# Kelvin-ywc/LPI

Hardware: AMD Instinct MI355X
Metric: image-text pairs/sec fwd+bwd (ViT-B/16, bs256/GPU) (higher is better)
Workload: dtype bf16; 1 GPU; BASELINE.json configs[2]: ViT-B/16 dual encoder bs=256/GPU prompt_depth=3 r=4 P=16, fwd+bwd incl. DecomposedPrompt grads + SGD step; global_batch=256, image=224x224, towers=lock step, GEMMs of one layer op grouped in one launch, parallelism=dp1, weights=synthetic (numpy Philox, CLIP-init scales), frozen

## Files before the change

### lpi_amd/csrc/gemm256p.hip

```cpp
#include "gemm256x128_tile.h"

extern int g_lpi_tuning[16];

namespace {

constexpr int T256 = 256;
constexpr int ROWB = 128;
constexpr int HALF_BYTES = 128 * ROWB;
constexpr int BUF_BYTES = 4 * HALF_BYTES;
constexpr int NTHR = 512;
constexpr int OFF_A0 = 0, OFF_A1 = HALF_BYTES, OFF_B0 = 2 * HALF_BYTES, OFF_B1 = 3 * HALF_BYTES;
constexpr int STG = BUF_BYTES;
constexpr int LDS_P = 2 * BUF_BYTES;
constexpr int EPI_PLAIN16 = 100;
template <int EPI, bool SAVE_U> constexpr bool slices_ok() { return !(EPI == LPI_EPI_QUICKGELU && SAVE_U); }

struct PProb {
    const void* A; const void* B; void* C; const float* bias; const void* residual; void* aux;
    int N, K, lda, ldb, ldc, ldr, ldaux, tiles_m, tiles_n;
    int vb0;
    int bias_off;
    int group_m;
};
struct PGroup {
    PProb p[2];
    int nprob;
    int n_full;
    int tail_blocks;
    int reserved;
    float alpha;
};

#ifdef LPI_GEMM_STAMPS
__device__ unsigned long long g_gemm_stamps[1024][8];
#define GS_NOW() __builtin_amdgcn_s_memtime()
#endif

template <typename T, typename TC, int EPI, bool RES, bool SAVE_U>
__global__ __launch_bounds__(NTHR, 2) void gemm256p_kernel(const PGroup grp)
{
    extern __shared__ __attribute__((aligned(16))) char smem[];
    constexpr int EPC = Elem<T>::EPC;
    constexpr int BK = ROWB / (int)sizeof(T);
    const int tid = threadIdx.x;
    const int lane = tid & 63;
    const int wave = __builtin_amdgcn_readfirstlane(tid >> 6);
    const int wm = wave >> 2, wn = wave & 3;
    const int G = gridDim.x;
    int group_m = 1;
    const float alpha = grp.alpha;
    typedef typename AuxT<T>::type TA;
    typedef float f32x8 __attribute__((ext_vector_type(8)));
    constexpr bool LNE = EPI == LPI_EPI_LN || EPI == LPI_EPI_LN_QUICKGELU;
    constexpr bool SLICES = slices_ok<EPI, SAVE_U>();
    constexpr bool P16 = EPI == EPI_PLAIN16;
    constexpr int EPIX = P16 ? LPI_EPI_NONE : EPI;
    const T* A = nullptr; const T* B = nullptr; TC* C = nullptr;
    const float* bias = nullptr; const float* residual = nullptr; TA* aux = nullptr;
    int K = 0, lda = 0, ldb = 0, ldc = 0, ldr = 0, ldaux = 0, tiles_m = 1, tiles_n = 1, nwg = 0, vb0 = 0, bias_off = 0;
    unsigned a_off = 0, b_off = 0;
    const int srow = tid >> 3;
    const int schunk = (tid & 7) ^ ((tid >> 4) & 7);
    auto bind = [&](int pi) {
        const PProb& P = grp.p[pi];
        A = (const T*)P.A; B = (const T*)P.B; C = (TC*)P.C; bias = P.bias; residual = (const float*)P.residual; aux = (TA*)P.aux;
        K = P.K; lda = P.lda; ldb = P.ldb; ldc = P.ldc; ldr = P.ldr; ldaux = P.ldaux; tiles_m = P.tiles_m; tiles_n = P.tiles_n;
        nwg = tiles_m * tiles_n; vb0 = P.vb0; bias_off = P.bias_off; group_m = P.group_m;
        a_off = (unsigned)(((size_t)srow * lda + schunk * EPC) * sizeof(T));
        b_off = (unsigned)(((size_t)srow * ldb + schunk * EPC) * sizeof(T));
    };

    auto coords = [&](int vb, int& m0, int& n0) {
        const int q = nwg >> 3, r = nwg & 7, xcd = vb & 7, idx = vb >> 3;
        const int t = (xcd < r ? xcd * (q + 1) : r * (q + 1) + (xcd - r) * q) + idx;
        const int gm = SLICES ? (group_m & 0xffff) : group_m;
        const int group = t / (gm * tiles_n);
        const int first_m = group * gm;
        const int gsz = min(tiles_m - first_m, gm);
        const int in_group = t - group * gm * tiles_n;
        m0 = (first_m + in_group % gsz) * T256;
        n0 = (in_group / gsz) * T256;
        if constexpr (SLICES) {
            const int wrap = (group_m >> 16) * T256;
            if (wrap) {
                if (m0 >= wrap) { m0 -= wrap; n0 += tiles_n * T256; }
                if (m0 >= wrap) { m0 -= wrap; n0 += tiles_n * T256; }
            }
        }
    };

    const unsigned lds_w = __builtin_amdgcn_readfirstlane((unsigned)(uintptr_t)(__attribute__((address_space(3))) char*)smem + wave * 1024);
    auto glds16 = [&](const T* sbase, unsigned voff, unsigned lds_addr) {
        unsigned keep;
        asm volatile("s_mov_b32 %0, m0\n\ts_mov_b32 m0, %3\n\ts_nop 0\n\tglobal_load_lds_dwordx4 %1, %2\n\ts_mov_b32 m0, %0"
                     : "=&s"(keep) : "v"(voff), "s"(sbase), "s"(lds_addr) : "memory");
    };
#ifndef LPI_A_POLICY
#define LPI_A_POLICY ""
#endif
    auto glds16a = [&](const T* sbase, unsigned voff, unsigned lds_addr) {
        unsigned keep;
        asm volatile("s_mov_b32 %0, m0\n\ts_mov_b32 m0, %3\n\ts_nop 0\n\tglobal_load_lds_dwordx4 %1, %2" LPI_A_POLICY "\n\ts_mov_b32 m0, %0"
                     : "=&s"(keep) : "v"(voff), "s"(sbase), "s"(lds_addr) : "memory");
    };
    auto stage_A = [&](int m0, int kt, int h, int buf) {
        const T* sb = A + (size_t)(m0 + h * 128) * lda + (size_t)kt * BK;
        const int lo = buf * BUF_BYTES + (h ? OFF_A1 : OFF_A0);
        glds16a(sb, a_off, lds_w + lo);
        glds16a(sb + (size_t)64 * lda, a_off, lds_w + lo + 8192);
    };
    auto stage_B = [&](int n0, int kt, int h, int buf) {
        const T* sb = B + (size_t)(n0 + h * 128) * ldb + (size_t)kt * BK;
        const int lo = buf * BUF_BYTES + (h ? OFF_B1 : OFF_B0);
        glds16(sb, b_off, lds_w + lo);
        glds16(sb + (size_t)64 * ldb, b_off, lds_w + lo + 8192);
    };

    const int frow = lane & 15, fg = lane >> 4, fsw = frow >> 1;
    int foff[2];
#pragma unroll
    for (int ks = 0; ks < 2; ++ks) foff[ks] = frow * ROWB + (((ks << 2) | fg) ^ fsw) * 16;
    const int a_base = (wm * 64) * ROWB;
    const int b_base = (wn * 32) * ROWB;

    Chunk fa[4][2], fb0[2][2], fb1[2][2];
    f32x4 acc[2][2][2][4];
    auto read_A = [&](const char* half) {
#pragma unroll
        for (int mi = 0; mi < 4; ++mi)
#pragma unroll
            for (int ks = 0; ks < 2; ++ks) fa[mi][ks].u = *reinterpret_cast<const uint4*>(half + a_base + mi * 16 * ROWB + foff[ks]);
    };
    auto read_B = [&](Chunk (&fb)[2][2], const char* half) {
#pragma unroll
        for (int ni = 0; ni < 2; ++ni)
#pragma unroll
            for (int ks = 0; ks < 2; ++ks) fb[ni][ks].u = *reinterpret_cast<const uint4*>(half + b_base + ni * 16 * ROWB + foff[ks]);
    };
    auto mma_quadrant = [&](f32x4 (&c)[2][2][2][4], int nh, int mh, const Chunk (&fb)[2][2]) {
        __builtin_amdgcn_s_setprio(1);
#pragma unroll
        for (int ks = 0; ks < 2; ++ks)
#pragma unroll
            for (int ni = 0; ni < 2; ++ni)
#pragma unroll
                for (int mi = 0; mi < 4; ++mi) mma_chunk<T>(c[nh][ni][mh][mi], fb[ni][ks], fa[mi][ks]);
        __builtin_amdgcn_s_setprio(0);
    };
#define PHASE_SYNC_IN()                                   \
    asm volatile("s_waitcnt lgkmcnt(0)" ::: "memory");    \
    __builtin_amdgcn_s_barrier();                         \
    __builtin_amdgcn_sched_barrier(0)
#define PHASE_SYNC_OUT()                                  \
    __builtin_amdgcn_sched_barrier(0);                    \
    __builtin_amdgcn_s_barrier();                         \
    asm volatile("" ::: "memory")

    int nk = 0;
    constexpr bool LATE = RES || EPI == LPI_EPI_DQUICKGELU;
    constexpr bool SIDE16 = (RES && sizeof(TC) == 2) || EPI == LPI_EPI_DQUICKGELU;
    constexpr bool STATS = EPI == LPI_EPI_NONE && RES && SAVE_U && __is_same(TC, f16_t);
    constexpr int NST = 8 + (STATS ? 2 : 0);
    const char* side_base = nullptr;
    int side_ld = 0;
    float* const bias_lds = reinterpret_cast<float*>(smem + LDS_P);
    if constexpr (SIDE16) {
        for (int pi = 0; pi < grp.nprob; ++pi) {
            const float* bp = grp.p[pi].bias;
            float* dst = bias_lds + grp.p[pi].bias_off;
            for (int i = tid * 4; i < grp.p[pi].N; i += NTHR * 4)
                *reinterpret_cast<f32x4*>(dst + i) = bp ? *reinterpret_cast<const f32x4*>(bp + i) : f32x4{0.f, 0.f, 0.f, 0.f};
        }
        __syncthreads();
    }
    auto stage_side = [&](int m0, int n0, int p) {
        const char* sb = side_base + ((size_t)m0 * side_ld + n0) * 2;
        int l2 = lane;
        asm volatile("" : "+v"(l2));
#pragma unroll
        for (int i = 0; i < 4; ++i) {
            const int sr = 2 * (4 * wave + i) + (l2 >> 5);
            const int trow = (p >> 1) * 128 + (sr >> 5) * 64 + ((p & 1) * 2 + ((sr >> 4) & 1)) * 16 + (sr & 15);
            const unsigned voff = (unsigned)trow * (unsigned)side_ld * 2u + (unsigned)(l2 & 31) * 16u;
            unsigned keep;
            asm volatile("s_mov_b32 %0, m0\n\ts_mov_b32 m0, %3\n\ts_nop 0\n\tglobal_load_lds_dwordx4 %1, %2 nt\n\ts_mov_b32 m0, %0"
                         : "=&s"(keep) : "v"(voff), "s"(sb), "s"(lds_w + (p & 1) * 32768 + i * 1024 + wave * 3072) : "memory");
        }
    };

#ifdef LPI_GEMM_STAMPS
    unsigned long long gs_main = 0, gs_epi = 0, gs_next = 0, gs_tiles = 0, gs_t0 = 0, gs_t1 = 0, gs_t2 = 0;
    unsigned long long gs_e[4] = {0, 0, 0, 0}, gs_a = 0, gs_b = 0;
#endif
    const int n_full = grp.n_full;
    int vbv = blockIdx.x;
    bool lds_used = false;
    for (int pi = 0; pi < grp.nprob; ++pi) {
        bind(pi);
        nk = K / BK;
        if constexpr (SIDE16) {
            side_base = RES ? reinterpret_cast<const char*>(residual) : reinterpret_cast<const char*>(aux);
            side_ld = RES ? ldr : ldaux;
        }
        const int vend = min(vb0 + nwg, n_full);
        if (vbv < vb0) vbv += (vb0 - vbv + G - 1) / G * G;
        if (vbv >= vend) continue;
        if (lds_used) {
            asm volatile("s_waitcnt lgkmcnt(0)" ::: "memory");
            __builtin_amdgcn_s_barrier();
            asm volatile("" ::: "memory");
        }
        lds_used = true;
        int vb = vbv - vb0;
        const int lend = vend - vb0;
        int m0, n0;
        coords(vb, m0, n0);
        m0 = __builtin_amdgcn_readfirstlane(m0);
        n0 = __builtin_amdgcn_readfirstlane(n0);
        stage_A(m0, 0, 0, 0); stage_B(n0, 0, 0, 0); stage_B(n0, 0, 1, 0); stage_A(m0, 0, 1, 0);
        stage_A(m0, 1, 0, 1); stage_B(n0, 1, 0, 1); stage_B(n0, 1, 1, 1);
        asm volatile("s_waitcnt vmcnt(8)" ::: "memory");
        __builtin_amdgcn_s_barrier();
        bool first = true;
        for (;;) {
            const int nvb = vb + G;
            const bool more_tiles = nvb < lend;
            const bool has_next = more_tiles && !LATE;
            int nm0 = 0, nn0 = 0;
            if (more_tiles) coords(nvb, nm0, nn0);
            nm0 = __builtin_amdgcn_readfirstlane(nm0);
            nn0 = __builtin_amdgcn_readfirstlane(nn0);
#pragma unroll
            for (int a = 0; a < 2; ++a)
#pragma unroll
                for (int b = 0; b < 2; ++b)
#pragma unroll
                    for (int c = 0; c < 2; ++c)
#pragma unroll
                        for (int d = 0; d < 4; ++d) acc[a][b][c][d] = f32x4{0.f, 0.f, 0.f, 0.f};
            if (wm == 1) __builtin_amdgcn_s_barrier();

            auto ktile = [&](int kt, const int BUF, bool skip_wait) {
                const char* buf = smem + BUF * BUF_BYTES;
                const bool more1 = kt + 1 < nk, more2 = kt + 2 < nk;
                read_B(fb0, buf + OFF_B0);
                read_B(fb1, buf + OFF_B1);
                __builtin_amdgcn_sched_barrier(0);
                read_A(buf + OFF_A0);
                if (more1) {
                    stage_A(m0, kt + 1, 1, BUF ^ 1);
                    if (!skip_wait) asm volatile("s_waitcnt vmcnt(8)" ::: "memory");
                } else if (has_next) {
                    stage_A(nm0, 0, 1, BUF ^ 1);
                    asm volatile("s_waitcnt vmcnt(8)" ::: "memory");
                } else {
                    asm volatile("s_waitcnt vmcnt(0)" ::: "memory");
                    if constexpr (SIDE16) {
                        stage_side(m0, n0, 0);
                        stage_side(m0, n0, 1);
                    }
                }
                PHASE_SYNC_IN();
                mma_quadrant(acc, 0, 0, fb0);
                mma_quadrant(acc, 1, 0, fb1);
                PHASE_SYNC_OUT();
                read_A(buf + OFF_A1);
                if (more2) {
                    stage_A(m0, kt + 2, 0, BUF); stage_B(n0, kt + 2, 0, BUF); stage_B(n0, kt + 2, 1, BUF);
                    asm volatile("s_waitcnt vmcnt(8)" ::: "memory");
                } else if (more1) {
                    if (has_next) {
                        stage_A(nm0, 0, 0, BUF); stage_B(nn0, 0, 0, BUF); stage_B(nn0, 0, 1, BUF);
                        asm volatile("s_waitcnt vmcnt(8)" ::: "memory");
                    } else {
                        asm volatile("s_waitcnt vmcnt(2)" ::: "memory");
                    }
                } else if (!has_next && !SIDE16) {
                    asm volatile("s_waitcnt vmcnt(0)" ::: "memory");
                }
                PHASE_SYNC_IN();
                mma_quadrant(acc, 1, 1, fb1);
                mma_quadrant(acc, 0, 1, fb0);
                PHASE_SYNC_OUT();
            };
#ifdef LPI_GEMM_STAMPS
            gs_t0 = GS_NOW();
            if (gs_tiles) gs_next += gs_t0 - gs_t2;
#endif
            ktile(0, 0, !first);
            ktile(1, 1, false);
            for (int kt = 2; kt < nk; kt += 2) {
                ktile(kt, 0, false);
                ktile(kt + 1, 1, false);
            }
            if (wm == 0) __builtin_amdgcn_s_barrier();
#ifdef LPI_GEMM_STAMPS
            gs_t1 = GS_NOW();
            gs_main += gs_t1 - gs_t0;
#endif

            int lane_e = lane, wave_e = wave;
            asm volatile("" : "+v"(lane_e));
            asm volatile("" : "+s"(wave_e));
            const int lrow = lane_e & 15, lslot = lane_e >> 4;
            const int wm_e = wave_e >> 2, wn_e = wave_e & 3;
            if constexpr (P16) {
                typedef __attribute__((ext_vector_type(4))) unsigned u32x4_;
                const int l5 = lane_e & 31, lh = lane_e >> 5;
                TC* const cbase = C + (size_t)m0 * ldc + n0 + l5 * 8;
#pragma unroll
                for (int p = 0; p < 4; ++p) {
                    const int mh = p >> 1;
                    char* const sb = smem + STG + (p & 1) * 32768;
#pragma unroll
                    for (int mi2 = 0; mi2 < 2; ++mi2) {
                        const int s_row = wm_e * 32 + mi2 * 16 + lrow;
#pragma unroll
                        for (int nh = 0; nh < 2; ++nh)
#pragma unroll
                            for (int ni = 0; ni < 2; ++ni) {
                                const int c8 = nh * 32 + wn_e * 8 + ni * 4 + lslot;
                                const f32x4 a = acc[nh][ni][mh][(p & 1) * 2 + mi2] + 0.0f;
                                *reinterpret_cast<uint2*>(sb + s_row * 512 + ((c8 ^ (2 * lrow)) << 3)) = uint2{pack2_t<TC>(a[0], a[1]), pack2_t<TC>(a[2], a[3])};
                            }
                    }
                    asm volatile("s_waitcnt lgkmcnt(0)" ::: "memory");
                    __builtin_amdgcn_s_barrier();
                    asm volatile("" ::: "memory");
#pragma unroll
                    for (int i = 0; i < 4; ++i) {
                        const int s_row = wave_e * 8 + 2 * i + lh;
                        const int trow = mh * 128 + (s_row >> 5) * 64 + ((p & 1) * 2 + ((s_row >> 4) & 1)) * 16 + (s_row & 15);
                        const u32x4_ v = *reinterpret_cast<const u32x4_*>(sb + s_row * 512 + (((2 * l5) ^ (2 * (s_row & 15))) << 3));
                        if constexpr (LPI_NTC_DEFAULT) __builtin_nontemporal_store(v, reinterpret_cast<u32x4_*>(cbase + (size_t)trow * ldc));
                        else *reinterpret_cast<u32x4_*>(cbase + (size_t)trow * ldc) = v;
                    }
                    if (p == 1 && has_next) asm volatile("s_waitcnt vmcnt(8)" ::: "memory");
                }
            } else {
            const int ecol = n0 + lane_e * 4;
            f32x4 bv = f32x4{0.f, 0.f, 0.f, 0.f};
            if constexpr (SIDE16) bv = *reinterpret_cast<const f32x4*>(bias_lds + bias_off + ecol);
            else if (bias) bv = *reinterpret_cast<const f32x4*>(bias + ecol);
            f32x4 c1v = f32x4{0.f, 0.f, 0.f, 0.f};
            if constexpr (EPI == LPI_EPI_LN || EPI == LPI_EPI_LN_QUICKGELU) c1v = *reinterpret_cast<const f32x4*>(residual + 2 * (size_t)ldr + ecol);
            char* const stg = smem + STG;
#pragma unroll
            for (int p = 0; p < 4; ++p) {
                const int mh = p >> 1;
#ifdef LPI_GEMM_STAMPS
                gs_a = GS_NOW();
#endif
                if (p) {
                    asm volatile("s_waitcnt lgkmcnt(0)" ::: "memory");
                    __builtin_amdgcn_s_barrier();
                }
#ifdef LPI_GEMM_STAMPS
                gs_b = GS_NOW(); gs_e[0] += gs_b - gs_a;
#endif
                if constexpr (SIDE16) {
                    if (p >= 1 && p <= 2) stage_side(m0, n0, p + 1);
                    if (p == 3 && more_tiles) { stage_A(nm0, 0, 0, 0); stage_A(nm0, 0, 1, 0); }
                }
                f32x8 mu8, rs8;
                if constexpr (LNE) {
                    const int sr0 = wave_e * 8;
                    const int trow0 = mh * 128 + (sr0 >> 5) * 64 + ((p & 1) * 2 + ((sr0 >> 4) & 1)) * 16 + (sr0 & 15);
                    const float* pm = residual + (m0 + trow0);
                    const float* pr = pm + ldr;
                    asm volatile("s_load_dwordx8 %0, %2, 0x0\n\ts_load_dwordx8 %1, %3, 0x0" : "=&s"(mu8), "=&s"(rs8) : "s"(pm), "s"(pr));
                }
#pragma unroll
                for (int mi2 = 0; mi2 < 2; ++mi2) {
                    const int s_row = wm_e * 32 + mi2 * 16 + lrow;
#pragma unroll
                    for (int nh = 0; nh < 2; ++nh)
#pragma unroll
                        for (int ni = 0; ni < 2; ++ni) {
                            const int chunk = nh * 32 + wn_e * 8 + ni * 4 + lslot;
                            *reinterpret_cast<f32x4*>(stg + s_row * 1024 + ((chunk ^ (s_row & 7)) << 4)) = acc[nh][ni][mh][(p & 1) * 2 + mi2];
                        }
                }
                if constexpr (SIDE16) {
                    if (p == 0) asm volatile("s_waitcnt vmcnt(4)" ::: "memory");
                    else if (p == 3 && !more_tiles) asm volatile("s_waitcnt vmcnt(%0)" :: "n"(NST) : "memory");
                    else asm volatile("s_waitcnt vmcnt(%0)" :: "n"(NST + 4) : "memory");
                }
                if constexpr (LNE) asm volatile("s_waitcnt lgkmcnt(0)" : "+s"(mu8), "+s"(rs8) : : "memory");
                else asm volatile("s_waitcnt lgkmcnt(0)" ::: "memory");
#ifdef LPI_GEMM_STAMPS
                gs_a = GS_NOW(); gs_e[1] += gs_a - gs_b;
#endif
                __builtin_amdgcn_s_barrier();
                asm volatile("" ::: "memory");
#ifdef LPI_GEMM_STAMPS
                gs_b = GS_NOW(); gs_e[2] += gs_b - gs_a;
#endif
                float st_s[8], st_q[8];
#pragma unroll
                for (int rr = 0; rr < 8; ++rr) {
                    const int s_row = wave_e * 8 + rr;
                    const int trow = mh * 128 + (s_row >> 5) * 64 + ((p & 1) * 2 + ((s_row >> 4) & 1)) * 16 + (s_row & 15);
                    const f32x4 v = *reinterpret_cast<const f32x4*>(stg + s_row * 1024 + ((lane_e ^ (s_row & 7)) << 4));
                    if constexpr (SIDE16) {
                        f32x4 o = v * alpha + bv;
                        const char* sp = smem + (p & 1) * 32768 + s_row * 512 + lane_e * 8;
                        if constexpr (EPI == LPI_EPI_DQUICKGELU) {
                            const f32x4 u = Elem<TA>::ld4(reinterpret_cast<const TA*>(sp));
                            o *= u;
                        } else {
                            o += Elem<TC>::ld4(reinterpret_cast<const TC*>(sp));
                        }
                        if constexpr (STATS) {
                            const uint32_t w0 = pack2_t<f16_t>(o[0], o[1]), w1 = pack2_t<f16_t>(o[2], o[3]);
                            *reinterpret_cast<uint2*>(C + (size_t)(m0 + trow) * ldc + ecol) = uint2{w0, w1};
                            f16x4_sum_sumsq(w0, w1, st_s[rr], st_q[rr]);
                        } else {
                            if constexpr (LPI_NTC_DEFAULT && EPI == LPI_EPI_DQUICKGELU) st4_nt<TC>(C + (size_t)(m0 + trow) * ldc + ecol, o);
                            else Elem<TC>::st4(C + (size_t)(m0 + trow) * ldc + ecol, o);
                        }
                    } else {
                        gemm_epilogue_store<T, TC, EPI, RES, SAVE_U>(v, m0 + trow, ecol, C, ldc, bv, alpha, residual, ldr, aux, ldaux, c1v, LNE ? mu8[rr] : 0.f,
                                                                     LNE ? rs8[rr] : 1.f);
                    }
                }
                if constexpr (STATS) {
                    float so, qo;
                    rowstats8_half_reduce(st_s, st_q, lane_e, so, qo);
                    const int s_row = wave_e * 8 + ((lane_e >> 2) & 7);
                    const int trow = mh * 128 + (s_row >> 5) * 64 + ((p & 1) * 2 + ((s_row >> 4) & 1)) * 16 + (s_row & 15);
                    float* sp = reinterpret_cast<float*>(aux) + (size_t)(2 * ((n0 >> 7) + (lane_e >> 5))) * ldaux + (m0 + trow);
                    if ((lane_e & 3) == 0) { sp[0] = so; sp[ldaux] = qo; }
                }
#ifdef LPI_GEMM_STAMPS
                gs_a = GS_NOW(); gs_e[3] += gs_a - gs_b;
#endif
                if (p == 1 && has_next) asm volatile("s_waitcnt vmcnt(16)" ::: "memory");
                if constexpr (LATE && !SIDE16) {
                    if (p == 1 && more_tiles) {
                        stage_A(nm0, 0, 0, 0); stage_B(nn0, 0, 0, 0); stage_B(nn0, 0, 1, 0); stage_A(nm0, 0, 1, 0);
                    }
                    if (p == 3 && more_tiles) asm volatile("s_waitcnt vmcnt(16)" ::: "memory");
                }
            }
            }
#ifdef LPI_GEMM_STAMPS
            gs_t2 = GS_NOW();
            gs_epi += gs_t2 - gs_t1;
            ++gs_tiles;
#endif
            if (!more_tiles) { vbv = nvb + vb0; break; }
            asm volatile("s_waitcnt lgkmcnt(0)" ::: "memory");
            __builtin_amdgcn_s_barrier();
            asm volatile("" ::: "memory");
            vb = nvb; m0 = nm0; n0 = nn0;
            if constexpr (SIDE16) {
                stage_B(n0, 0, 0, 0); stage_B(n0, 0, 1, 0);
                stage_A(m0, 1, 0, 1); stage_B(n0, 1, 0, 1); stage_B(n0, 1, 1, 1);
                asm volatile("s_waitcnt vmcnt(6)" ::: "memory");
                __builtin_amdgcn_s_barrier();
            } else {
                stage_A(m0, 1, 0, 1); stage_B(n0, 1, 0, 1); stage_B(n0, 1, 1, 1);
                first = false;
            }
        }
    }
#undef PHASE_SYNC_IN
#undef PHASE_SYNC_OUT

#ifdef LPI_GEMM_STAMPS
    if (tid == 0 && blockIdx.x < 1024) {
        g_gemm_stamps[blockIdx.x][0] = gs_main; g_gemm_stamps[blockIdx.x][1] = gs_epi; g_gemm_stamps[blockIdx.x][2] = gs_next; g_gemm_stamps[blockIdx.x][3] = gs_tiles;
        for (int i = 0; i < 4; ++i) g_gemm_stamps[blockIdx.x][4 + i] = gs_e[i];
    }
#endif
    if (grp.tail_blocks > 0) {
        for (int j = blockIdx.x; j < grp.tail_blocks; j += G) {
            const int k = (j >> 4) * 8 + (j & 7), half = (j >> 3) & 1;
            const int v = n_full + k;
            const int pi = (grp.nprob > 1 && v >= grp.p[1].vb0) ? 1 : 0;
            bind(pi);
            const int lv = v - vb0;
            if (lv < 0 || lv >= nwg) continue;
            __syncthreads();
            int m0, n0;
            coords(lv, m0, n0);
            t128::tile<T, TC, EPIX, RES, SAVE_U>(m0, n0 + half * 128, K, A, lda, B, ldb, C, ldc, bias, residual, ldr, aux, ldaux, alpha, smem);
        }
    }
}

int cu_count_p() { return lpi_cu_count(); }

struct HostProb {
    int M, N, K;
    const void* A; int lda; const void* B; int ldb; void* C; int ldc; const float* bias; const float* residual; int ldr; void* aux; int ldaux;
};

template <typename T, typename TC, int EPI, bool RES, bool SAVE_U>
int launchp_impl(const HostProb* hp, int np, float alpha, hipStream_t s)
{
    constexpr bool SIDE16 = (RES && sizeof(TC) == 2) || EPI == LPI_EPI_DQUICKGELU;
    static_assert(EPI != EPI_PLAIN16 || (!RES && !SAVE_U && sizeof(TC) == 2), "EPI_PLAIN16: store-only, 2-byte output");
    const int ncu = cu_count_p();
    PGroup g = {};
    g.nprob = np;
    g.alpha = alpha;
    int v = 0, nsum = 0;
    for (int i = 0; i < np; ++i) {
        PProb& P = g.p[i];
        const HostProb& h = hp[i];
        P.A = h.A; P.B = h.B; P.C = h.C; P.bias = h.bias; P.residual = h.residual; P.aux = h.aux;
        P.N = h.N; P.K = h.K; P.lda = h.lda; P.ldb = h.ldb; P.ldc = h.ldc; P.ldr = h.ldr; P.ldaux = h.ldaux;
        P.tiles_m = h.M / T256; P.tiles_n = h.N / T256;
        P.vb0 = v;
        v += P.tiles_m * P.tiles_n;
        P.bias_off = nsum;
        P.group_m = g_lpi_tuning[4] > 0 ? g_lpi_tuning[4] : ((size_t)h.N * h.K * sizeof(T) <= ((size_t)5 << 20) ? 1 : 8);
        if (slices_ok<EPI, SAVE_U>() && P.group_m == 1 && g_lpi_tuning[15] >= 0 && P.tiles_m < 32768) {
            int S = 0;
            const size_t wbytes = (size_t)h.N * h.K * sizeof(T);
            if (g_lpi_tuning[15] > 0) S = g_lpi_tuning[15];
            else if (wbytes > ((size_t)3 << 20) && P.tiles_n % 2 == 0) S = 2;
            if ((S == 2 || S == 3) && P.tiles_n % S == 0 && P.tiles_n / S >= 2) {
                P.group_m |= P.tiles_m << 16;
                P.tiles_n /= S;
                P.tiles_m *= S;
            }
        }
        nsum += h.N;
    }
    if (SIDE16 && nsum > 8192) return LPI_ENOSYS;
    const int rem = v % ncu;
    g.n_full = v;
    if (g_lpi_tuning[6] != 0 && v - rem >= ncu && rem > 0 && rem <= ncu / 2 && (ncu % 8) == 0) {
        g.n_full = v - rem;
        g.tail_blocks = 16 * ((rem + 7) >> 3);
    }
    auto kern = gemm256p_kernel<T, TC, EPI, RES, SAVE_U>;
    const int LDS = std::max<int>(t128::LDS_BYTES, LDS_P + (SIDE16 ? nsum * 4 : 0));
    static LdsOnce once;
    if (int e = lpi_ensure_lds(once, (const void*)kern, 160 * 1024)) return e;
    lpi_note_gemm_kernel(g.tail_blocks ? LPI_GEMM_K_256_TAIL : LPI_GEMM_K_256);
    const int grid = std::min(ncu, std::max(g.n_full, g.tail_blocks));
    LPI_LAUNCH(kern, dim3(grid), dim3(NTHR), LDS, s, g);
    LPI_CHECK_LAST();
    return 0;
}

template <typename T, typename TC>
int dispatchp(int epi, const HostProb* hp, int np, float alpha, hipStream_t s)
{
    const bool res = hp[0].residual != nullptr, ax = hp[0].aux != nullptr;
    for (int i = 1; i < np; ++i)
        if ((hp[i].residual != nullptr) != res || (hp[i].aux != nullptr) != ax) return LPI_EINVAL;
    switch (epi) {
    case LPI_EPI_NONE:
        if (res) return launchp_impl<T, TC, LPI_EPI_NONE, true, false>(hp, np, alpha, s);
        if constexpr (sizeof(TC) == 2) {
            bool plain = alpha == 1.0f && !ax && g_lpi_tuning[14] != 1;
            for (int i = 0; i < np; ++i) plain = plain && hp[i].bias == nullptr;
            if (plain) return launchp_impl<T, TC, EPI_PLAIN16, false, false>(hp, np, alpha, s);
        }
        return launchp_impl<T, TC, LPI_EPI_NONE, false, false>(hp, np, alpha, s);
    case LPI_EPI_RES_ROWSTATS:
        if constexpr (sizeof(TC) == 2 && !__is_same(TC, bf16_t)) {
            if (!res || !ax) return LPI_EINVAL;
            return launchp_impl<T, TC, LPI_EPI_NONE, true, true>(hp, np, alpha, s);
        }
        return LPI_ENOSYS;
    case LPI_EPI_QUICKGELU:
        if (res) return LPI_ENOSYS;
        if (ax) return launchp_impl<T, TC, LPI_EPI_QUICKGELU, false, true>(hp, np, alpha, s);
        return launchp_impl<T, TC, LPI_EPI_QUICKGELU, false, false>(hp, np, alpha, s);
    case LPI_EPI_DQUICKGELU:
        if (res) return LPI_ENOSYS;
        if (!ax) return LPI_EINVAL;
        return launchp_impl<T, TC, LPI_EPI_DQUICKGELU, false, false>(hp, np, alpha, s);
    }
    return LPI_EINVAL;
}

template <typename T, typename TC>
int dispatchp_ln(int epi, const HostProb* hp, int np, float alpha, hipStream_t s)
{
    const bool ax = hp[0].aux != nullptr;
    for (int i = 0; i < np; ++i)
        if (!hp[i].residual || (hp[i].aux != nullptr) != ax) return LPI_EINVAL;
    if (epi == LPI_EPI_LN) {
        if (ax) return LPI_EINVAL;
        return launchp_impl<T, TC, LPI_EPI_LN, false, false>(hp, np, alpha, s);
    }
    if (ax) return launchp_impl<T, TC, LPI_EPI_LN_QUICKGELU, false, true>(hp, np, alpha, s);
    return launchp_impl<T, TC, LPI_EPI_LN_QUICKGELU, false, false>(hp, np, alpha, s);
}

int launch_group(int dtype, int c_dtype, int epilogue, const HostProb* hp, int np, float alpha, hipStream_t s)
{
    if (epilogue == LPI_EPI_LN || epilogue == LPI_EPI_LN_QUICKGELU) {
        if (dtype == LPI_F16 && c_dtype == LPI_BF16) return dispatchp_ln<f16_t, bf16_t>(epilogue, hp, np, alpha, s);
        if (dtype == LPI_F16 && c_dtype == LPI_F16) return dispatchp_ln<f16_t, f16_t>(epilogue, hp, np, alpha, s);
        if (dtype == LPI_BF16 && c_dtype == LPI_BF16) return dispatchp_ln<bf16_t, bf16_t>(epilogue, hp, np, alpha, s);
        return LPI_ENOSYS;
    }
    if (dtype == LPI_BF16 && c_dtype == LPI_BF16) return dispatchp<bf16_t, bf16_t>(epilogue, hp, np, alpha, s);
    if (dtype == LPI_BF16 && c_dtype == LPI_F32) return dispatchp<bf16_t, float>(epilogue, hp, np, alpha, s);
    if (dtype == LPI_BF16 && c_dtype == LPI_F16 && (epilogue == LPI_EPI_NONE || epilogue == LPI_EPI_RES_ROWSTATS) && hp[0].residual) {
        for (int i = 1; i < np; ++i) if (!hp[i].residual) return LPI_EINVAL;
        if (epilogue == LPI_EPI_RES_ROWSTATS) {
            for (int i = 0; i < np; ++i) if (!hp[i].aux) return LPI_EINVAL;
            return launchp_impl<bf16_t, f16_t, LPI_EPI_NONE, true, true>(hp, np, alpha, s);
        }
        return launchp_impl<bf16_t, f16_t, LPI_EPI_NONE, true, false>(hp, np, alpha, s);
    }
    if (dtype == LPI_F16 && c_dtype == LPI_F16) return dispatchp<f16_t, f16_t>(epilogue, hp, np, alpha, s);
    if (dtype == LPI_F16 && c_dtype == LPI_F32) return dispatchp<f16_t, float>(epilogue, hp, np, alpha, s);
    return LPI_ENOSYS;
}

}

#ifdef LPI_GEMM_STAMPS
extern "C" int lpi_gemm_stamps_read(unsigned long long* dst) {
    return (int)hipMemcpyFromSymbol(dst, HIP_SYMBOL(g_gemm_stamps), sizeof(unsigned long long) * 1024 * 8, 0, hipMemcpyDeviceToHost);
}
#endif

int lpi_gemm256p_launch(int dtype, int c_dtype, int M, int N, int K, const void* A, int lda, const void* B, int ldb, void* C, int ldc,
                        const float* bias, const float* residual, int ldr, int epilogue, void* aux, int ldaux, float alpha, hipStream_t s)
{
    const HostProb hp = {M, N, K, A, lda, B, ldb, C, ldc, bias, residual, ldr, aux, ldaux};
    return launch_group(dtype, c_dtype, epilogue, &hp, 1, alpha, s);
}

int lpi_gemm256p_launch2(int dtype, int c_dtype, int epilogue, float alpha, const lpi_gemm_desc* d, hipStream_t s)
{
    HostProb hp[2];
    for (int i = 0; i < 2; ++i)
        hp[i] = HostProb{d[i].M, d[i].N, d[i].K, d[i].A, d[i].lda, d[i].B, d[i].ldb, d[i].C, d[i].ldc, d[i].bias, (const float*)d[i].residual, d[i].ldr,
                         d[i].aux, d[i].ldaux};
    return launch_group(dtype, c_dtype, epilogue, hp, 2, alpha, s);
}
```

Before: 11410 pairs/s.

## Load residual/aux side tiles into registers and prefetch next tile during SIDE16 epilogue

Residual and dQuickGELU side inputs used to be staged through LDS with global_load_lds. They are now loaded straight into registers with nontemporal loads, spread across the last k-tile, the post-mainloop point and the epilogue rows. The SIDE16 path no longer uses the LATE schedule, so the next tile's A/B operands prefetch during the main loop as in the plain path, and the separate restage-and-barrier at tile change is dropped. The k-loop is restructured with explicit position tags, and bias loading into LDS is skipped when there is no bias. The changes aim to hide side-input latency and cut barriers and LDS traffic, at the cost of extra VGPRs (16 u32x2 per thread) and hand-tuned vmcnt counts that must exactly match the new load order.

```diff
diff --git a/lpi_amd/csrc/gemm256p.hip b/lpi_amd/csrc/gemm256p.hip
--- a/lpi_amd/csrc/gemm256p.hip
+++ b/lpi_amd/csrc/gemm256p.hip
@@ -157,35 +157,32 @@
     asm volatile("" ::: "memory")
 
     int nk = 0;
-    constexpr bool LATE = RES || EPI == LPI_EPI_DQUICKGELU;
+    constexpr bool LATE = RES && sizeof(TC) == 4;
     constexpr bool SIDE16 = (RES && sizeof(TC) == 2) || EPI == LPI_EPI_DQUICKGELU;
     constexpr bool STATS = EPI == LPI_EPI_NONE && RES && SAVE_U && __is_same(TC, f16_t);
     constexpr int NST = 8 + (STATS ? 2 : 0);
+    constexpr int NSL = SIDE16 ? 8 : 0;
     const char* side_base = nullptr;
     int side_ld = 0;
     float* const bias_lds = reinterpret_cast<float*>(smem + LDS_P);
     if constexpr (SIDE16) {
         for (int pi = 0; pi < grp.nprob; ++pi) {
             const float* bp = grp.p[pi].bias;
+            if (!bp) continue;
             float* dst = bias_lds + grp.p[pi].bias_off;
-            for (int i = tid * 4; i < grp.p[pi].N; i += NTHR * 4)
-                *reinterpret_cast<f32x4*>(dst + i) = bp ? *reinterpret_cast<const f32x4*>(bp + i) : f32x4{0.f, 0.f, 0.f, 0.f};
+            for (int i = tid * 4; i < grp.p[pi].N; i += NTHR * 4) *reinterpret_cast<f32x4*>(dst + i) = *reinterpret_cast<const f32x4*>(bp + i);
         }
         __syncthreads();
     }
-    auto stage_side = [&](int m0, int n0, int p) {
-        const char* sb = side_base + ((size_t)m0 * side_ld + n0) * 2;
-        int l2 = lane;
-        asm volatile("" : "+v"(l2));
-#pragma unroll
-        for (int i = 0; i < 4; ++i) {
-            const int sr = 2 * (4 * wave + i) + (l2 >> 5);
-            const int trow = (p >> 1) * 128 + (sr >> 5) * 64 + ((p & 1) * 2 + ((sr >> 4) & 1)) * 16 + (sr & 15);
-            const unsigned voff = (unsigned)trow * (unsigned)side_ld * 2u + (unsigned)(l2 & 31) * 16u;
-            unsigned keep;
-            asm volatile("s_mov_b32 %0, m0\n\ts_mov_b32 m0, %3\n\ts_nop 0\n\tglobal_load_lds_dwordx4 %1, %2 nt\n\ts_mov_b32 m0, %0"
-                         : "=&s"(keep) : "v"(voff), "s"(sb), "s"(lds_w + (p & 1) * 32768 + i * 1024 + wave * 3072) : "memory");
-        }
+    typedef unsigned u32x2_ __attribute__((ext_vector_type(2)));
+    struct SideRegs { u32x2_ r[8]; };
+    SideRegs sd[2];
+    const unsigned side_loff = (unsigned)lane * 8u;
+    auto load_side_row = [&](int m0, int n0, int p, int rr) -> u32x2_ {
+        const int s_row = wave * 8 + rr;
+        const int trow = (p >> 1) * 128 + (s_row >> 5) * 64 + ((p & 1) * 2 + ((s_row >> 4) & 1)) * 16 + (s_row & 15);
+        const char* sb = side_base + ((size_t)(m0 + trow) * side_ld + n0) * 2;
+        return __builtin_nontemporal_load(reinterpret_cast<const u32x2_*>(sb + side_loff));
     };
 
 #ifdef LPI_GEMM_STAMPS
@@ -240,35 +237,33 @@
                         for (int d = 0; d < 4; ++d) acc[a][b][c][d] = f32x4{0.f, 0.f, 0.f, 0.f};
             if (wm == 1) __builtin_amdgcn_s_barrier();
 
-            auto ktile = [&](int kt, const int BUF, bool skip_wait) {
+            auto ktile = [&](int kt, const int BUF, const int POS, bool skip_wait) {
                 const char* buf = smem + BUF * BUF_BYTES;
-                const bool more1 = kt + 1 < nk, more2 = kt + 2 < nk;
                 read_B(fb0, buf + OFF_B0);
                 read_B(fb1, buf + OFF_B1);
                 __builtin_amdgcn_sched_barrier(0);
                 read_A(buf + OFF_A0);
-                if (more1) {
+                if (POS < 2) {
                     stage_A(m0, kt + 1, 1, BUF ^ 1);
                     if (!skip_wait) asm volatile("s_waitcnt vmcnt(8)" ::: "memory");
-                } else if (has_next) {
-                    stage_A(nm0, 0, 1, BUF ^ 1);
-                    asm volatile("s_waitcnt vmcnt(8)" ::: "memory");
                 } else {
-                    asm volatile("s_waitcnt vmcnt(0)" ::: "memory");
+                    if (has_next) stage_A(nm0, 0, 1, BUF ^ 1);
                     if constexpr (SIDE16) {
-                        stage_side(m0, n0, 0);
-                        stage_side(m0, n0, 1);
+#pragma unroll
+                        for (int rr = 0; rr < 8; ++rr) sd[0].r[rr] = load_side_row(m0, n0, 0, rr);
                     }
+                    if (has_next) asm volatile("s_waitcnt vmcnt(%0)" :: "n"(8 + NSL) : "memory");
+                    else asm volatile("s_waitcnt vmcnt(%0)" :: "n"(NSL) : "memory");
                 }
                 PHASE_SYNC_IN();
                 mma_quadrant(acc, 0, 0, fb0);
                 mma_quadrant(acc, 1, 0, fb1);
                 PHASE_SYNC_OUT();
                 read_A(buf + OFF_A1);
-                if (more2) {
+                if (POS == 0) {
                     stage_A(m0, kt + 2, 0, BUF); stage_B(n0, kt + 2, 0, BUF); stage_B(n0, kt + 2, 1, BUF);
                     asm volatile("s_waitcnt vmcnt(8)" ::: "memory");
-                } else if (more1) {
+                } else if (POS == 1) {
                     if (has_next) {
                         stage_A(nm0, 0, 0, BUF); stage_B(nn0, 0, 0, BUF); stage_B(nn0, 0, 1, BUF);
                         asm volatile("s_waitcnt vmcnt(8)" ::: "memory");
@@ -287,13 +282,19 @@
             gs_t0 = GS_NOW();
             if (gs_tiles) gs_next += gs_t0 - gs_t2;
 #endif
-            ktile(0, 0, !first);
-            ktile(1, 1, false);
-            for (int kt = 2; kt < nk; kt += 2) {
-                ktile(kt, 0, false);
-                ktile(kt + 1, 1, false);
+            bool skip = !first;
+            for (int kt = 0; kt < nk - 2; kt += 2) {
+                ktile(kt, 0, 0, skip);
+                ktile(kt + 1, 1, 0, false);
+                skip = false;
             }
+            ktile(nk - 2, 0, 1, skip);
+            ktile(nk - 1, 1, 2, false);
             if (wm == 0) __builtin_amdgcn_s_barrier();
+            if constexpr (SIDE16) {
+#pragma unroll
+                for (int rr = 0; rr < 8; ++rr) sd[1].r[rr] = load_side_row(m0, n0, 1, rr);
+            }
 #ifdef LPI_GEMM_STAMPS
             gs_t1 = GS_NOW();
             gs_main += gs_t1 - gs_t0;
@@ -340,7 +341,7 @@
             } else {
             const int ecol = n0 + lane_e * 4;
             f32x4 bv = f32x4{0.f, 0.f, 0.f, 0.f};
-            if constexpr (SIDE16) bv = *reinterpret_cast<const f32x4*>(bias_lds + bias_off + ecol);
+            if constexpr (SIDE16) { if (bias) bv = *reinterpret_cast<const f32x4*>(bias_lds + bias_off + ecol); }
             else if (bias) bv = *reinterpret_cast<const f32x4*>(bias + ecol);
             f32x4 c1v = f32x4{0.f, 0.f, 0.f, 0.f};
             if constexpr (EPI == LPI_EPI_LN || EPI == LPI_EPI_LN_QUICKGELU) c1v = *reinterpret_cast<const f32x4*>(residual + 2 * (size_t)ldr + ecol);
@@ -358,10 +359,6 @@
 #ifdef LPI_GEMM_STAMPS
                 gs_b = GS_NOW(); gs_e[0] += gs_b - gs_a;
 #endif
-                if constexpr (SIDE16) {
-                    if (p >= 1 && p <= 2) stage_side(m0, n0, p + 1);
-                    if (p == 3 && more_tiles) { stage_A(nm0, 0, 0, 0); stage_A(nm0, 0, 1, 0); }
-                }
                 f32x8 mu8, rs8;
                 if constexpr (LNE) {
                     const int sr0 = wave_e * 8;
@@ -382,9 +379,10 @@
                         }
                 }
                 if constexpr (SIDE16) {
-                    if (p == 0) asm volatile("s_waitcnt vmcnt(4)" ::: "memory");
-                    else if (p == 3 && !more_tiles) asm volatile("s_waitcnt vmcnt(%0)" :: "n"(NST) : "memory");
-                    else asm volatile("s_waitcnt vmcnt(%0)" :: "n"(NST + 4) : "memory");
+                    if (p == 0) asm volatile("s_waitcnt vmcnt(8)" ::: "memory");
+                    else if (p == 1) asm volatile("s_waitcnt vmcnt(%0)" :: "n"(NST + 8) : "memory");
+                    else if (p == 2) asm volatile("s_waitcnt vmcnt(%0)" :: "n"(2 * NST) : "memory");
+                    else asm volatile("s_waitcnt vmcnt(%0)" :: "n"(2 * NST - 8) : "memory");
                 }
                 if constexpr (LNE) asm volatile("s_waitcnt lgkmcnt(0)" : "+s"(mu8), "+s"(rs8) : : "memory");
                 else asm volatile("s_waitcnt lgkmcnt(0)" ::: "memory");
@@ -404,12 +402,12 @@
                     const f32x4 v = *reinterpret_cast<const f32x4*>(stg + s_row * 1024 + ((lane_e ^ (s_row & 7)) << 4));
                     if constexpr (SIDE16) {
                         f32x4 o = v * alpha + bv;
-                        const char* sp = smem + (p & 1) * 32768 + s_row * 512 + lane_e * 8;
+                        const u32x2_ sv = sd[p & 1].r[rr];
                         if constexpr (EPI == LPI_EPI_DQUICKGELU) {
-                            const f32x4 u = Elem<TA>::ld4(reinterpret_cast<const TA*>(sp));
+                            const f32x4 u = Elem<TA>::ld4(reinterpret_cast<const TA*>(&sv));
                             o *= u;
                         } else {
-                            o += Elem<TC>::ld4(reinterpret_cast<const TC*>(sp));
+                            o += Elem<TC>::ld4(reinterpret_cast<const TC*>(&sv));
                         }
                         if constexpr (STATS) {
                             const uint32_t w0 = pack2_t<f16_t>(o[0], o[1]), w1 = pack2_t<f16_t>(o[2], o[3]);
@@ -419,6 +417,7 @@
                             if constexpr (LPI_NTC_DEFAULT && EPI == LPI_EPI_DQUICKGELU) st4_nt<TC>(C + (size_t)(m0 + trow) * ldc + ecol, o);
                             else Elem<TC>::st4(C + (size_t)(m0 + trow) * ldc + ecol, o);
                         }
+                        if (p < 2) sd[p & 1].r[rr] = load_side_row(m0, n0, p + 2, rr);
                     } else {
                         gemm_epilogue_store<T, TC, EPI, RES, SAVE_U>(v, m0 + trow, ecol, C, ldc, bv, alpha, residual, ldr, aux, ldaux, c1v, LNE ? mu8[rr] : 0.f,
                                                                      LNE ? rs8[rr] : 1.f);
@@ -435,8 +434,8 @@
 #ifdef LPI_GEMM_STAMPS
                 gs_a = GS_NOW(); gs_e[3] += gs_a - gs_b;
 #endif
-                if (p == 1 && has_next) asm volatile("s_waitcnt vmcnt(16)" ::: "memory");
-                if constexpr (LATE && !SIDE16) {
+                if (p == 1 && has_next && !SIDE16) asm volatile("s_waitcnt vmcnt(16)" ::: "memory");
+                if constexpr (LATE) {
                     if (p == 1 && more_tiles) {
                         stage_A(nm0, 0, 0, 0); stage_B(nn0, 0, 0, 0); stage_B(nn0, 0, 1, 0); stage_A(nm0, 0, 1, 0);
                     }
@@ -454,15 +453,8 @@
             __builtin_amdgcn_s_barrier();
             asm volatile("" ::: "memory");
             vb = nvb; m0 = nm0; n0 = nn0;
-            if constexpr (SIDE16) {
-                stage_B(n0, 0, 0, 0); stage_B(n0, 0, 1, 0);
-                stage_A(m0, 1, 0, 1); stage_B(n0, 1, 0, 1); stage_B(n0, 1, 1, 1);
-                asm volatile("s_waitcnt vmcnt(6)" ::: "memory");
-                __builtin_amdgcn_s_barrier();
-            } else {
-                stage_A(m0, 1, 0, 1); stage_B(n0, 1, 0, 1); stage_B(n0, 1, 1, 1);
-                first = false;
-            }
+            stage_A(m0, 1, 0, 1); stage_B(n0, 1, 0, 1); stage_B(n0, 1, 1, 1);
+            first = false;
         }
     }
 #undef PHASE_SYNC_IN
```

New measurement: 11330 pairs/s. Within noise of the previous version (-0.7%).
